# Sudaraka88/LDWeaver

Hardware: AMD Instinct MI355X
Metric: MI SNP-pairs/sec (higher is better)
Workload: dtype i8

## Files before the change

ldweaver_amd/csrc/ldw_apx.hip:

```cpp
#include <algorithm>
#include <cmath>
#include <cstdlib>
#include <cstring>

#include "ldw_apx.h"
#include "ldw_dev.h"

using namespace ldw;

namespace ldw {

namespace {
constexpr int64_t APX_PROD_CAP = 12000;
struct ProdTable {
    std::vector<int32_t> val;
    std::vector<uint8_t> a, b;
    ProdTable() {
        std::vector<std::pair<int32_t, std::pair<uint8_t, uint8_t>>> all;
        for (int x = 0; x <= 127; ++x)
            for (int y = x; y <= 127; ++y) all.push_back({x * y, {(uint8_t)x, (uint8_t)y}});
        std::sort(all.begin(), all.end());
        for (auto &e : all)
            if (val.empty() || val.back() != e.first) {
                val.push_back(e.first);
// ... 724 lines not shown
                for (int i = 0; i < MT; ++i)
#pragma unroll
                    for (int j = 0; j < NT; ++j)
#pragma unroll
                        for (int e = 0; e < 16; ++e) acc[i][j][e] = (int)((unsigned)acc[i][j][e] >> sh);
            }
        };
        exp_issue(wcur[1], 2 * m + 1);
        rescale(sh4.x);
        if (wave_live) kstep(tile0, 0);
        exp_finish(wdst + 32768);
        rescale(sh4.y);
        if (wave_live) kstep(tile0, 1);
        __syncthreads();
        if (m + 1 < P.M2) exp_issue(wnext[0], 2 * m + 2);
        rescale(sh4.z);
        if (wave_live) kstep(tile0 + 32768, 0);
        if (m + 1 < P.M2) exp_finish(wdst);
        rescale(sh4.w);
        if (wave_live) kstep(tile0 + 32768, 1);
        __syncthreads();
        wcur = wnext;
        wnext = wfar;
    }
    if (!wave_live) return;
    apx_gemm_epilogue<MT, NT>(P, acc, ty, tx, lane, s_tab, reinterpret_cast<uint8_t *>(s_tab + 64 * 64) + wave * 256);
}

#endif

int launch_apx_live_tiles(ldw_ctx *c, const ApxGemmArgs &P, hipStream_t st) {
    LDW_REQUIRE(P.fuse && P.skip_ctr && P.tile_list && P.n_live && P.RTpad % 128 == 0 && P.RFpad % 64 == 0 && P.tab && P.tab_nb == 64,
                LDW_ERR_ARG, "launch_apx_live_tiles: bad pruning arguments");
    hipLaunchKernelGGL(k_apx_live_tiles, dim3((unsigned)(P.RTpad / (32 * APX_MT))), dim3(256), 0, st, P);
    LDW_HIP(hipGetLastError());
    return LDW_OK;
}

int launch_gemm_apx(ldw_ctx *c, const ApxGemmArgs &P, hipStream_t st) {
    LDW_REQUIRE(P.RTpad % APX_TW == 0 && P.RFpad % APX_TW == 0 && P.M2 > 0, LDW_ERR_ARG, "launch_gemm_apx: padding violated (RT %d RF %d M2 %d)", P.RTpad,
                P.RFpad, P.M2);
    const size_t lds = APX_LUT_BYTES + (size_t)P.M2 * 256 + (P.fuse ? (size_t)P.tab_nb * P.tab_nb * 8 + 1024 : 0);
    LDW_REQUIRE(lds <= 65536, LDW_ERR_ARG, "launch_gemm_apx: %d positions do not fit the LDS digit arrays", P.M2 * 128);
    LDW_REQUIRE(!P.fuse || (P.tab_nb == 64 && P.bin_t && P.bin_f && P.tab && P.clean), LDW_ERR_ARG, "launch_gemm_apx: bad table arguments");
    static const int tile = [] {
        const char *e = exp_env("LDW_APX_TILE");
        return e ? atoi(e) : 42;
    }();
#ifdef LDW_EXPERIMENTS
    const int kern = apx_kernel_is_lds() ? 1 : 0;
    static const bool pipe = [] { const char *e = exp_env("LDW_APX_KERNEL"); return e && e[0] == 'p'; }();
    if (pipe && !P.fine && tile == 42) {
        const int ntx = P.RFpad / 64, nty = P.RTpad / 128;
        hipLaunchKernelGGL(gemm_apx_pipe_kernel, dim3((unsigned)((ntx + 1) / 2), (unsigned)((nty + 1) / 2)), dim3(256), lds, st, P);
        LDW_HIP(hipGetLastError());
        int64_t waves = 0;
        for (int ty = 0; ty < nty; ++ty) {
            if (!P.lower_only) waves += ntx;
            else for (int tx = 0; tx < ntx; ++tx) waves += (tx * 64 + 63 < ty * 128) ? 0 : 1;
        }
        c->gemm_stat[0] += 1;
        if (P.fuse) c->gemm_stat[5] += 1;
        c->gemm_stat[1] += 2.0 * (double)waves * 128 * 64 * ((double)P.M2 * 128.0);
        return LDW_OK;
    }
    const size_t lds2 = 2048 + (size_t)P.M2 * 256 + 2 * 32768 + (P.fuse ? (size_t)P.tab_nb * P.tab_nb * 8 + 8 * 256 : 0);
    if (kern == 1 && lds2 <= 160 * 1024 && tile == 42) {
        static bool attr_set = false;
        if (!attr_set) {
            LDW_HIP(hipFuncSetAttribute(reinterpret_cast<const void *>(gemm_apx_lds_kernel), hipFuncAttributeMaxDynamicSharedMemorySize, 160 * 1024));
            attr_set = true;
        }
        const int ntx = P.RFpad / 64, nty = P.RTpad / 128;
        hipLaunchKernelGGL(gemm_apx_lds_kernel, dim3((unsigned)((ntx + 3) / 4), (unsigned)((nty + 1) / 2)), dim3(512), lds2, st, P);
        LDW_HIP(hipGetLastError());
        int64_t waves = 0;
        for (int ty = 0; ty < nty; ++ty) {
            if (!P.lower_only) waves += ntx;
            else for (int tx = 0; tx < ntx; ++tx) waves += (tx * 64 + 63 < ty * 128) ? 0 : 1;
        }
        c->gemm_stat[0] += 1;
        if (P.fuse) c->gemm_stat[5] += 1;
        c->gemm_stat[1] += 2.0 * (double)waves * 128 * 64 * ((double)P.M2 * 128.0);
        return LDW_OK;
    }
#endif
#define LDW_APX_LAUNCH(MTv, NTv)                                                                                              \
    {                                                                                                                         \
        const int ntx = P.RFpad / (32 * NTv), nty = P.RTpad / (32 * MTv);                                                     \
        if (P.fine) hipLaunchKernelGGL((gemm_apx_kernel<MTv, NTv, true>), dim3((unsigned)((ntx + 1) / 2), (unsigned)((nty + 1) / 2)), dim3(256), lds, st, P); \
        else hipLaunchKernelGGL((gemm_apx_kernel<MTv, NTv, false>), dim3((unsigned)((ntx + 1) / 2), (unsigned)((nty + 1) / 2)), dim3(256), lds, st, P); \
    }
    if (P.skip_ctr) {
        LDW_REQUIRE(P.fuse && P.tile_list && P.n_live && P.RFpad % 64 == 0, LDW_ERR_ARG, "launch_gemm_apx: bad pruning arguments");
        const int tiles = (P.RTpad / (32 * APX_MT)) * (P.RFpad / 64), g = (tiles + 3) / 4;
        if (P.fine) hipLaunchKernelGGL((gemm_apx_kernel<APX_MT, 2, true, APX_WPS>), dim3((unsigned)g), dim3(256), lds, st, P);
        else hipLaunchKernelGGL((gemm_apx_kernel<APX_MT, 2, false, APX_WPS>), dim3((unsigned)g), dim3(256), lds, st, P);
    }
#ifdef LDW_EXPERIMENTS
    else if (tile == 22 && !P.fuse) LDW_APX_LAUNCH(2, 2)
    else if (tile == 33 && !P.fuse) {
        const int ntx = (P.RFpad + 95) / 96, nty = (P.RTpad + 95) / 96;
        if (P.fine) hipLaunchKernelGGL((gemm_apx_kernel<3, 3, true, 2>), dim3((unsigned)((ntx + 1) / 2), (unsigned)((nty + 1) / 2)), dim3(256), lds, st, P);
        else hipLaunchKernelGGL((gemm_apx_kernel<3, 3, false, 2>), dim3((unsigned)((ntx + 1) / 2), (unsigned)((nty + 1) / 2)), dim3(256), lds, st, P);
    }
    else if (tile == 224 && !P.fuse) {
        const int ntx = P.RFpad / 64, nty = P.RTpad / 64;
        if (P.fine) hipLaunchKernelGGL((gemm_apx_kernel<2, 2, true, 4>), dim3((unsigned)((ntx + 1) / 2), (unsigned)((nty + 1) / 2)), dim3(256), lds, st, P);
        else hipLaunchKernelGGL((gemm_apx_kernel<2, 2, false, 4>), dim3((unsigned)((ntx + 1) / 2), (unsigned)((nty + 1) / 2)), dim3(256), lds, st, P);
    }
    else if (tile == 24 && !P.fuse) LDW_APX_LAUNCH(2, 4)
    else if (tile == 32 && !P.fuse) {
        const int ntx = P.RFpad / 64, nty = (P.RTpad + 95) / 96;
        if (P.fine) hipLaunchKernelGGL((gemm_apx_kernel<3, 2, true, 3>), dim3((unsigned)((ntx + 1) / 2), (unsigned)((nty + 1) / 2)), dim3(256), lds, st, P);
        else hipLaunchKernelGGL((gemm_apx_kernel<3, 2, false, 3>), dim3((unsigned)((ntx + 1) / 2), (unsigned)((nty + 1) / 2)), dim3(256), lds, st, P);
    }
#endif
    else LDW_APX_LAUNCH(4, 2)
#undef LDW_APX_LAUNCH
    LDW_HIP(hipGetLastError());
    {
        const int tl = P.fuse ? 42 : tile;
        const int MTv = (P.fuse && P.skip_ctr) ? APX_MT : (tl == 22 || tl == 24 || tl == 224 ? 2 : (tl == 32 || tl == 33 ? 3 : 4)), NTv = tl == 24 ? 4 : (tl == 33 ? 3 : 2), TH = 32 * MTv, TWd = 32 * NTv;
        int64_t waves = 0;
        for (int ty = 0; ty * TH < P.RTpad; ++ty) {
            const int ntx = P.RFpad / TWd;
            if (!P.lower_only) waves += ntx;
            else for (int tx = 0; tx < ntx; ++tx) waves += (tx * TWd + TWd - 1 < ty * TH) ? 0 : 1;
        }
        c->gemm_stat[0] += 1;
        if (P.fuse) c->gemm_stat[5] += 1;
        c->gemm_stat[1] += 2.0 * (double)waves * TH * TWd * ((double)P.M2 * 128.0);
        if (P.fuse && P.skip_ctr) {
            c->apx_ops_per_wave = 2.0 * TH * TWd * ((double)P.M2 * 128.0);
            c->apx_waves_total += waves;
        }
    }
    return LDW_OK;
}

struct PairArgs {
    const uint64_t *Mbits;
    int64_t KW;
    int nwords, path, nseg;
    int seg_in_lds;
    const PopSeg *segs;
    const int32_t *wbeg, *row0;
    int32_t zero_row;
    int64_t *sums;
    EpiArgs A;
    unsigned long long *ghist;
};

template <int CA, int CB>
__device__ __forceinline__ void pair_sums_body(const PairArgs &P, int path, const int32_t *s_wbeg, const PopSeg *s_segs) {
    constexpr bool GENB = CA == 4 && CB == 4;
    const EpiArgs &A = P.A;
    const int sub = path * PAIR_SHARDS + (int)blockIdx.y;
    unsigned int n = A.pl_n[sub];
    n = n > A.pl_cap ? A.pl_cap : n;
    const int lane = threadIdx.x & 63;
    const PairEnt *list = A.pl_pairs + (int64_t)sub * A.pl_cap;
    constexpr int KW = 3, KS = 2;
    uint32_t smask[KW][KS];
    int64_t sV[KW][KS];
    bool more[KW];
#pragma unroll
    for (int k = 0; k < KW; ++k) {
        const int w = lane + 64 * k;
        int s0 = 0, s1 = 0;
        if (w < P.nwords) {
            s0 = s_wbeg[w] & 0x7FFFFFFF;
            s1 = s_wbeg[w + 1] & 0x7FFFFFFF;
        }
        more[k] = s1 - s0 > KS;
#pragma unroll
        for (int q = 0; q < KS; ++q) {
            const bool on = s0 + q < s1 && !more[k];
            smask[k][q] = on ? s_segs[s0 + q].mask : 0u;
            sV[k][q] = on ? s_segs[s0 + q].V : 0;
        }
    }
    for (unsigned int idx = blockIdx.x * 4u + (threadIdx.x >> 6); idx < n; idx += gridDim.x * 4u) {
        const PairEnt e = list[idx];
        const uint32_t era = (uint32_t)__builtin_amdgcn_readfirstlane((int)e.ra), erb = (uint32_t)__builtin_amdgcn_readfirstlane((int)e.rb);
        const int r0a = (int)(era & 0x1FFFFFFFu), na = (int)(era >> 29), r0b = (int)(erb & 0x1FFFFFFFu), nb = (int)(erb >> 29);
        const uint32_t *fr[CA], *tr[CB];
#pragma unroll
        for (int i = 0; i < CA; ++i) fr[i] = reinterpret_cast<const uint32_t *>(P.Mbits + (int64_t)(i < na ? r0a + i : P.zero_row) * P.KW);
#pragma unroll
        for (int j = 0; j < CB; ++j) tr[j] = reinterpret_cast<const uint32_t *>(P.Mbits + (int64_t)(j < nb ? r0b + j : P.zero_row) * P.KW);
        int64_t s[CB][CA];
#pragma unroll
        for (int j = 0; j < CB; ++j)
#pragma unroll
            for (int i = 0; i < CA; ++i) s[j][i] = 0;
        uint32_t f[KW][CA], tt[KW][CB];
#pragma unroll
        for (int k = 0; k < KW; ++k) {
            const int w = lane + 64 * k;
            const bool in = w < P.nwords;
#pragma unroll
            for (int i = 0; i < CA; ++i) f[k][i] = (in && (!GENB || i < na)) ? fr[i][w] : 0u;
#pragma unroll
            for (int j = 0; j < CB; ++j) tt[k][j] = (in && (!GENB || j < nb)) ? tr[j][w] : 0u;
        }
#pragma unroll
        for (int k = 0; k < KW; ++k) {
            if (more[k]) {
                const int w = lane + 64 * k;
                const int s0 = s_wbeg[w] & 0x7FFFFFFF, s1 = s_wbeg[w + 1] & 0x7FFFFFFF;
                for (int sg = s0; sg < s1; ++sg) {
                    const PopSeg seg = s_segs[sg];
#pragma unroll
                    for (int j = 0; j < CB; ++j)
#pragma unroll
                        for (int i = 0; i < CA; ++i)
                            if (!GENB || (i < na && j < nb)) s[j][i] += (int64_t)((uint64_t)__popc(f[k][i] & tt[k][j] & seg.mask) * (uint64_t)seg.V);
                }
            } else {
#pragma unroll
                for (int q2 = 0; q2 < KS; ++q2)
#pragma unroll
                    for (int j = 0; j < CB; ++j)
#pragma unroll
                        for (int i = 0; i < CA; ++i)
                            if (!GENB || (i < na && j < nb)) s[j][i] += (int64_t)((uint64_t)__popc(f[k][i] & tt[k][j] & smask[k][q2]) * (uint64_t)sV[k][q2]);
            }
        }
        for (int w = lane + 64 * KW; w < P.nwords; w += 64) {
            uint32_t f2[CA], t2[CB];
#pragma unroll
            for (int i = 0; i < CA; ++i) f2[i] = (!GENB || i < na) ? fr[i][w] : 0u;
#pragma unroll
            for (int j = 0; j < CB; ++j) t2[j] = (!GENB || j < nb) ? tr[j][w] : 0u;
            const int s0 = s_wbeg[w] & 0x7FFFFFFF, s1 = s_wbeg[w + 1] & 0x7FFFFFFF;
            for (int sg = s0; sg < s1; ++sg) {
                const PopSeg seg = s_segs[sg];
#pragma unroll
                for (int j = 0; j < CB; ++j)
#pragma unroll
                    for (int i = 0; i < CA; ++i)
                        if (!GENB || (i < na && j < nb)) s[j][i] += (int64_t)((uint64_t)__popc(f2[i] & t2[j] & seg.mask) * (uint64_t)seg.V);
            }
        }
#pragma unroll
        for (int j = 0; j < CB; ++j)
#pragma unroll
            for (int i = 0; i < CA; ++i) {
                int64_t v = s[j][i];
                if (!GENB || (i < na && j < nb)) {
#pragma unroll
                    for (int off = 32; off > 0; off >>= 1) v += __shfl_xor(v, off);
                }
                if (lane == 0) P.sums[((int64_t)sub * A.pl_cap + idx) * 16 + j * 4 + i] = v;
            }
    }
}

template <bool GEN>
__global__ __launch_bounds__(256) void k_pair_sums(PairArgs P) {
    extern __shared__ __attribute__((aligned(16))) uint8_t pop_smem[];
    int32_t *s_wbeg = reinterpret_cast<int32_t *>(pop_smem);
    PopSeg *s_segs = reinterpret_cast<PopSeg *>(pop_smem + (((size_t)P.nwords + 4) * 4 + 15) / 16 * 16);
    const int path = GEN ? 4 : (int)blockIdx.z;
    if (blockIdx.x * 4u >= P.A.pl_n[path * PAIR_SHARDS + (int)blockIdx.y]) return;
    if (P.seg_in_lds) {
        for (int i = threadIdx.x; i < P.nwords + 1; i += 256) s_wbeg[i] = P.wbeg[i];
        for (int i = threadIdx.x; i < P.nseg; i += 256) s_segs[i] = P.segs[i];
        __syncthreads();
    } else {
        s_wbeg = const_cast<int32_t *>(P.wbeg);
        s_segs = const_cast<PopSeg *>(P.segs);
    }
    if constexpr (GEN) {
        pair_sums_body<4, 4>(P, 4, s_wbeg, s_segs);
    } else {
        switch (path) {
            case 0: pair_sums_body<1, 1>(P, 0, s_wbeg, s_segs); break;
            case 1: pair_sums_body<2, 1>(P, 1, s_wbeg, s_segs); break;
            case 2: pair_sums_body<1, 2>(P, 2, s_wbeg, s_segs); break;
            default: pair_sums_body<2, 2>(P, 3, s_wbeg, s_segs); break;
        }
    }
}

template <int CA, int CB>
__device__ __forceinline__ void pair_sums_bits_body(const PairArgs &P, int path, const int64_t *sVT, int stride) {
    constexpr bool GENB = CA == 4 && CB == 4;
    const EpiArgs &A = P.A;
    const int sub = path * PAIR_SHARDS + (int)blockIdx.y;
    unsigned int n = A.pl_n[sub];
    n = n > A.pl_cap ? A.pl_cap : n;
    const int lane = threadIdx.x & 63;
    const PairEnt *list = A.pl_pairs + (int64_t)sub * A.pl_cap;
    for (unsigned int idx = blockIdx.x * 4u + (threadIdx.x >> 6); idx < n; idx += gridDim.x * 4u) {
        const PairEnt e = list[idx];
        const uint32_t era = (uint32_t)__builtin_amdgcn_readfirstlane((int)e.ra), erb = (uint32_t)__builtin_amdgcn_readfirstlane((int)e.rb);
        const int r0a = (int)(era & 0x1FFFFFFFu), na = (int)(era >> 29), r0b = (int)(erb & 0x1FFFFFFFu), nb = (int)(erb >> 29);
        const uint32_t *fr[CA], *tr[CB];
#pragma unroll
        for (int i = 0; i < CA; ++i) fr[i] = reinterpret_cast<const uint32_t *>(P.Mbits + (int64_t)(i < na ? r0a + i : P.zero_row) * P.KW);
#pragma unroll
        for (int j = 0; j < CB; ++j) tr[j] = reinterpret_cast<const uint32_t *>(P.Mbits + (int64_t)(j < nb ? r0b + j : P.zero_row) * P.KW);
        int64_t s[CB][CA];
#pragma unroll
        for (int j = 0; j < CB; ++j)
#pragma unroll
            for (int i = 0; i < CA; ++i) s[j][i] = 0;
        for (int w = lane; w < P.nwords; w += 64) {
            uint32_t f[CA], t[CB], uf = 0u, ut = 0u;
#pragma unroll
            for (int i = 0; i < CA; ++i) {
                f[i] = (!GENB || i < na) ? fr[i][w] : 0u;
                uf |= f[i];
            }
#pragma unroll
            for (int j = 0; j < CB; ++j) {
                t[j] = (!GENB || j < nb) ? tr[j][w] : 0u;
                ut |= t[j];
            }
            uint32_t u = uf & ut;
            while (u) {
                const int b = __builtin_ctz(u);
                u &= u - 1u;
                const int64_t v = sVT[b * stride + w];
#pragma unroll
                for (int j = 0; j < CB; ++j)
#pragma unroll
                    for (int i = 0; i < CA; ++i)
                        if (CA * CB == 1 || (((f[i] & t[j]) >> b) & 1u)) s[j][i] += v;
            }
        }
#pragma unroll
        for (int j = 0; j < CB; ++j)
#pragma unroll
            for (int i = 0; i < CA; ++i) {
                int64_t v = s[j][i];
                if (!GENB || (i < na && j < nb)) {
#pragma unroll
                    for (int off = 32; off > 0; off >>= 1) v += __shfl_xor(v, off);
                }
                if (lane == 0) P.sums[((int64_t)sub * A.pl_cap + idx) * 16 + j * 4 + i] = v;
            }
    }
}

template <bool GEN>
__global__ __launch_bounds__(256) void k_pair_sums_bits(PairArgs P, const int64_t *__restrict__ vpos, int stride) {
    extern __shared__ __attribute__((aligned(16))) uint8_t pop_smem[];
    int64_t *sVT = reinterpret_cast<int64_t *>(pop_smem);
    const int path = GEN ? 4 : (int)blockIdx.z;
    if (blockIdx.x * 4u >= P.A.pl_n[path * PAIR_SHARDS + (int)blockIdx.y]) return;
    for (int i = threadIdx.x; i < 32 * stride; i += 256) {
        const int b = i / stride, w = i - b * stride;
        sVT[i] = w < P.nwords ? vpos[32 * w + b] : 0;
    }
    __syncthreads();
    if constexpr (GEN) {
        pair_sums_bits_body<4, 4>(P, 4, sVT, stride);
    } else {
        switch (path) {
            case 0: pair_sums_bits_body<1, 1>(P, 0, sVT, stride); break;
            case 1: pair_sums_bits_body<2, 1>(P, 1, sVT, stride); break;
            case 2: pair_sums_bits_body<1, 2>(P, 2, sVT, stride); break;
            default: pair_sums_bits_body<2, 2>(P, 3, sVT, stride); break;
        }
    }
}

constexpr int PAIR_HWIN = 128;

template <int NA, int NB>
__device__ __forceinline__ void pair_mi_body(const PairArgs &P, int path, unsigned int *s_hist) {
    constexpr bool GEN = NA == 0;
    const EpiArgs &A = P.A;
    const EmitArgs &E = A.E;
    const int sub = path * PAIR_SHARDS + (int)blockIdx.y;
    unsigned int n = A.pl_n[sub];
    n = n > A.pl_cap ? A.pl_cap : n;
    const bool square = A.nf == A.nt;
    const PairEnt *list = A.pl_pairs + (int64_t)sub * A.pl_cap;
    const int lane = (int)(threadIdx.x & 63);
    for (unsigned int base = blockIdx.x * 256u + (threadIdx.x & ~63u); base < n; base += gridDim.x * 256u) {
        const unsigned int idx = base + (unsigned int)lane;
        bool valid = idx < n;
        uint32_t t = 0, q = 0;
        if (valid) {
            t = list[idx].t;
            q = list[idx].q;
        }
        const RowPack &RP = A.rowpack[t];
        valid = valid && RP.a_loc >= 0;
        bool cand = false;
        int bk = 0, seg = -1, a_loc = 0, b_loc = 0, sg = 0;
        double mi = 0.0;
        if (valid) {
            const RowSide R = RP.R;
            a_loc = RP.a_loc;
            const ColMeta M = A.colpack[q];
            b_loc = M.bl;
            sg = A.span ? M.ci.pad[0] : 0;
            const int64_t *sp = P.sums + ((int64_t)sub * A.pl_cap + idx) * 16;
            if constexpr (GEN) {
                mi = pair_mi<4, 4>(A, R, M, a_loc, b_loc, square, gacc_plain(sp, 1, 4));
            } else {
                mi = pair_mi_full<NA, NB>(A, R, M, a_loc, b_loc, square, gacc_plain(sp, 1, 4));
            }
            seg = pair_seg(a_loc, b_loc, E.lower_only);
            if (seg >= 0 && E.any_sr && col_is_sr(M.ci, a_loc)) {
                emit_pair_spec(E, M.ci, a_loc, b_loc, R.sa, M.sb, mi, P.ghist);
            } else if (seg >= 0 && E.do_lr && mi >= E.spec_lo) {
                bk = mi_bucket(mi);
                cand = bk >= E.spec_B;
            }
        }
        if (A.span) {
            for (int k = 0; k < A.span; ++k) {
                const bool mine = cand && sg == k;
                const unsigned long long mk = __ballot(mine);
                if (mk == 0ull) continue;
                const int leader = __builtin_ctzll(mk);
                unsigned long long pos = 0;
                if (lane == leader) pos = atomicAdd(A.sseg[k].n_cand, (unsigned long long)__popcll(mk));
                pos = __shfl(pos, leader);
                if (mine) {
                    pos += (unsigned long long)__popcll(mk & ((1ull << lane) - 1ull));
                    A.sseg[k].ckey[pos] = f64_key(mi);
                    A.sseg[k].cval[pos] = ((uint64_t)seg << 62) | ((uint64_t)a_loc + (uint64_t)b_loc * (uint64_t)E.nf);
                    const int w = bk - (E.spec_B > 0 ? E.spec_B : 0);
                    if (w < PAIR_HWIN) atomicAdd(&s_hist[k * PAIR_HWIN + w], 1u);
                    else atomicAdd(&A.sseg[k].ghist[bk], 1ull);
                }
            }
            continue;
        }
        const unsigned long long mk = __ballot(cand);
        if (mk == 0ull) continue;
        const int leader = __builtin_ctzll(mk);
        unsigned long long pos = 0;
        if (lane == leader) pos = atomicAdd(E.n_cand, (unsigned long long)__popcll(mk));
        pos = __shfl(pos, leader);
        if (cand) {
            pos += (unsigned long long)__popcll(mk & ((1ull << lane) - 1ull));
            E.ckey[pos] = f64_key(mi);
            E.cval[pos] = ((uint64_t)seg << 62) | ((uint64_t)a_loc + (uint64_t)b_loc * (uint64_t)E.nf);
            const int w = bk - (E.spec_B > 0 ? E.spec_B : 0);
            if (w < PAIR_HWIN) atomicAdd(&s_hist[w], 1u);
            else atomicAdd(&P.ghist[bk], 1ull);
        }
    }
}

__global__ __launch_bounds__(256) void k_pair_mi(PairArgs P) {
    __shared__ unsigned int s_hist[LDW_SPAN_MAX * PAIR_HWIN];
    for (int i = threadIdx.x; i < LDW_SPAN_MAX * PAIR_HWIN; i += 256) s_hist[i] = 0u;
    __syncthreads();
    switch (blockIdx.z) {
        case 0: pair_mi_body<1, 1>(P, 0, s_hist); break;
        case 1: pair_mi_body<2, 1>(P, 1, s_hist); break;
        case 2: pair_mi_body<1, 2>(P, 2, s_hist); break;
        case 3: pair_mi_body<2, 2>(P, 3, s_hist); break;
        default: pair_mi_body<0, 0>(P, 4, s_hist); break;
    }
    __syncthreads();
    const int hb0 = P.A.E.spec_B > 0 ? P.A.E.spec_B : 0;
    if (P.A.span) {
        for (int i = threadIdx.x; i < P.A.span * PAIR_HWIN; i += 256) {
            const int k = i / PAIR_HWIN, w = i - k * PAIR_HWIN;
            if (s_hist[i] != 0u && hb0 + w < NBINS) atomicAdd(&P.A.sseg[k].ghist[hb0 + w], (unsigned long long)s_hist[i]);
        }
        return;
    }
    if (threadIdx.x < PAIR_HWIN && s_hist[threadIdx.x] != 0u && hb0 + (int)threadIdx.x < NBINS)
        atomicAdd(&P.ghist[hb0 + threadIdx.x], (unsigned long long)s_hist[threadIdx.x]);
}

int launch_pairs_exact(ldw_ctx *c, const EpiArgs &A, unsigned long long *ghist, int64_t *sums, hipStream_t st) {
    PairArgs P;
    memset(&P, 0, sizeof(P));
    P.Mbits = c->Mbits.as<uint64_t>();
    P.KW = c->KW;
    P.nwords = (int)(c->KW * 2);
    P.nseg = c->n_pop_segs;
    P.segs = c->pop_segs.as<PopSeg>();
    P.wbeg = c->pop_wbeg.as<int32_t>();
    P.row0 = c->row0.as<int32_t>();
    P.zero_row = (int32_t)c->R;
    P.sums = sums;
    P.A = A;
    P.ghist = ghist;
    size_t lds = (((size_t)P.nwords + 4) * 4 + 15) / 16 * 16 + (size_t)P.nseg * sizeof(PopSeg);
    P.seg_in_lds = lds <= 60000 ? 1 : 0;
    if (!P.seg_in_lds) lds = 0;
    const int stride = (P.nwords + 31) / 32 * 32;
    const size_t lds_bits = (size_t)32 * stride * 8;
    const bool bits_off = getenv("LDW_NO_PAIR_BITS") != nullptr;
    const bool many_classes = !P.seg_in_lds || P.nseg >= 8 * P.nwords;
    if (many_classes && !bits_off && lds_bits <= 160 * 1024 && c->pop_vpos.p) {
        if (lds_bits > 64 * 1024 && !c->pair_bits_attr) {
            LDW_HIP(hipFuncSetAttribute(reinterpret_cast<const void *>(k_pair_sums_bits<false>), hipFuncAttributeMaxDynamicSharedMemorySize, 160 * 1024));
            LDW_HIP(hipFuncSetAttribute(reinterpret_cast<const void *>(k_pair_sums_bits<true>), hipFuncAttributeMaxDynamicSharedMemorySize, 160 * 1024));
            c->pair_bits_attr = true;
        }
        hipLaunchKernelGGL(k_pair_sums_bits<false>, dim3(256, PAIR_SHARDS, 4), dim3(256), lds_bits, st, P, c->pop_vpos.as<int64_t>(), stride);
        hipLaunchKernelGGL(k_pair_sums_bits<true>, dim3(256, PAIR_SHARDS, 1), dim3(256), lds_bits, st, P, c->pop_vpos.as<int64_t>(), stride);
    } else {
        static const unsigned gx_env = [] { const char *e = getenv("LDW_PAIR_GRID"); return e ? (unsigned)atoi(e) : 0u; }();
        hipLaunchKernelGGL(k_pair_sums<false>, dim3(gx_env ? gx_env : 512u, PAIR_SHARDS, 4), dim3(256), lds, st, P);
        hipLaunchKernelGGL(k_pair_sums<true>, dim3(gx_env ? gx_env : 1024u, PAIR_SHARDS, 1), dim3(256), lds, st, P);
    }
    hipLaunchKernelGGL(k_pair_mi, dim3(64, PAIR_SHARDS, PAIR_PATHS), dim3(256), 0, st, P);
    LDW_HIP(hipGetLastError());
    return LDW_OK;
}

}

namespace ldw {
void warm_apx() {
    hipFuncAttributes a;
    (void)hipFuncGetAttributes(&a, reinterpret_cast<const void *>(&k_pack_panel));
    (void)hipGetLastError();
}
}
```

ldweaver_amd/csrc/ldw_internal.h:

```cpp
#pragma once
#include <hip/hip_runtime.h>
#include <stdint.h>
#include <stdlib.h>
#include <string>
#include <atomic>
#include <memory>
#include <mutex>
#include <thread>
#include <vector>

#include "../../include/ldweaver_amd.h"

#define LDW_NSLOT 3

#ifdef LDW_EXPERIMENTS
#define LDW_HAS_EXPERIMENTS 1
#else
#define LDW_HAS_EXPERIMENTS 0
#endif

namespace ldw {

inline const char *exp_env(const char *name) {
#ifdef LDW_EXPERIMENTS
    return getenv(name);
#else
    (void)name;
    return nullptr;
#endif
}

void set_error(const char *fmt, ...);
int hip_fail(hipError_t e, const char *what, const char *file, int line);

#define LDW_HIP(call)                                                        \
    do {                                                                     \
        hipError_t e__ = (call);                                             \
        if (e__ != hipSuccess) return ldw::hip_fail(e__, #call, __FILE__, __LINE__); \
    } while (0)

#define LDW_REQUIRE(cond, code, ...)   \
    do {                               \
        if (!(cond)) {                 \
            ldw::set_error(__VA_ARGS__); \
            return (code);             \
        }                              \
    } while (0)

struct DevBuf {
    void *p = nullptr;
    size_t cap = 0;
    int reserve(size_t bytes);
    int reserve_keep(size_t bytes, size_t used, hipStream_t s);
    void release();
    template <class T> T *as() const { return reinterpret_cast<T *>(p); }
};

constexpr int TILE = 128;
constexpr int KSTEP = 128;
constexpr int NBINS = 4096;

struct BlockStat {
    int64_t n_lr_total = 0, n_lr_kept = 0, n_sr = 0;
    double disc_thresh = 0;
};
struct BlockTrace {
    int diag = 0, guess = -1, B_true = -1, margin = 0, path = 0 , missed = 0, probed = 0;
    long long n_cand = 0;
};

}

struct ldw_ctx {
    int device = 0;
    hipStream_t stream = nullptr;
    bool own_stream = true;
    hipEvent_t ev[6] = {nullptr, nullptr, nullptr, nullptr, nullptr, nullptr};
    double last_ms[4] = {0, 0, 0, 0};
    int engine = LDW_ENGINE_MFMA;

    int64_t L = 0, N = 0, Npad = 0;
    int64_t KW = 0;
    ldw::DevBuf states;
    ldw::DevBuf chars;
    int64_t cN = 0, cL = 0;
    void *fasta = nullptr;

    bool have_weights = false;
    int nlimbs = 5;
    int frac_bits = 0;
    double neff = 0;
    int64_t total_fixed = 0;
    ldw::DevBuf digits;
    ldw::DevBuf vfixed;
    std::vector<int64_t> h_vfixed;
    std::vector<int64_t> h_vfixed_hi;
    int64_t total_fixed_hi = 0;
    double lo_abs_sum = 0;
    int mixed = 1;

    std::vector<int32_t> h_seq_perm;
    ldw::DevBuf seq_perm;
    int path_mode = 0;
    int select_mode = 0;
    bool apx_ok = false;
    bool apx_fine = false;
    std::string apx_gate = "weights not set";
    ldw::DevBuf dig_a, dig_b;
    ldw::DevBuf apx_shift;
    int apx_e_last = 0;
    int apx_transitions = 0;
    double apx_lost_units = 0;
    double apx_delta = 0;
    std::vector<int64_t> h_vapx;
    ldw::DevBuf slot_papx;
    ldw::DevBuf pop_segs, pop_wbeg;
    ldw::DevBuf pop_vpos;
    bool pair_bits_attr = false;
    int n_pop_segs = 0, n_classes = 0;
    ldw::DevBuf panel[LDW_NSLOT][2];
    ldw::DevBuf Gapx[LDW_NSLOT];
    ldw::DevBuf tab11[2];
    double tab11_lo[2] = {0, 0};
    int tab11_cur[2] = {0, 0};
    int64_t tab11_builds = 0;
    float tab11_c = 0;
    int tab11_nb = 0;
    bool tab11_on = true;
    ldw::DevBuf pair_sums;
    ldw::DevBuf pairs[LDW_NSLOT];
    ldw::DevBuf sub_units[LDW_NSLOT], sub_packs[LDW_NSLOT], sub_bins[LDW_NSLOT], sub_live[LDW_NSLOT];
    ldw::DevBuf scr_live[LDW_NSLOT];
    ldw::DevBuf apx_bins[LDW_NSLOT], apx_clean[LDW_NSLOT];
    ldw::DevBuf apx_mini[LDW_NSLOT];
    ldw::DevBuf apx_units[LDW_NSLOT], apx_packs[LDW_NSLOT];
    int64_t apx_blocks = 0, apx_units_listed = 0, apx_pairs_listed = 0, probe_blocks = 0, generic_blocks = 0;
    bool prune = true;
    ldw::DevBuf apx_skip;
    double apx_ops_per_wave = 0;
    int64_t apx_waves_skipped = 0, apx_waves_total = 0;
    bool span_on = true;
    bool diag_split = false;
    bool span_corners = false;
    int span_max = 8;
    int64_t maybe_entries = 0;
    int64_t pair_list_overflows = 0, maybe_overflows = 0;
    bool maybe_off = false;
    int64_t span_items = 0, span_blocks = 0, span_fallbacks = 0;
    int64_t span_sr_subs = 0;
    bool early_sr = false;
    std::atomic<int64_t> sorted_blocks{0};
    std::mutex order_mtx;
    ldw::DevBuf snp_sup;
    double r_min = 0;
    struct OrderCache { std::vector<int32_t> idx, order; };
    std::vector<std::unique_ptr<OrderCache>> order_cache;

    bool have_meta = false;
    double g = 0;
    ldw::DevBuf r, uqe, POS, paint;
    std::vector<double> h_r;
    std::vector<int32_t> h_POS, h_paint;
    int32_t paint_min = 0, paint_max = 0;
    bool pos_sorted = true;
    bool pos_strict = true;
    ldw::DevBuf pos_slot;
    int64_t n_slots = 0;
    double sr_total_dist = -1;
    int64_t sr_total = -1;
    uint64_t sr_share_key = 0;
    int64_t sr_share_rows = -1;

    bool rows_ready = false;
    int64_t R = 0;
    ldw::DevBuf Mbits;
    ldw::DevBuf row0;
    ldw::DevBuf slot_meta;
    ldw::DevBuf slot_pfix;
    ldw::DevBuf slot_pfix_hi;
    bool hi_ready = false;
    ldw::DevBuf glo;
    ldw::DevBuf lo_rows;
    ldw::DevBuf packs;
    ldw::DevBuf counts;
    ldw::DevBuf pfix_state;
    std::vector<int32_t> h_row0;
    std::vector<uint32_t> h_slot_meta;
    std::vector<int32_t> h_counts;
    std::vector<int64_t> h_minor_w;
    std::vector<int32_t> h_span_bad;

    ldw::DevBuf G, G2, G3;
    ldw::DevBuf MIblk;
    ldw::DevBuf rowlist_f, rowlist_t, idx_f, idx_t, lrow_f, lrow_t, perm_f, perm_t;
    ldw::DevBuf epi_rest;
    ldw::DevBuf scr_units;
    ldw::DevBuf hist[LDW_NSLOT], cand_key[LDW_NSLOT], cand_val[LDW_NSLOT];
    ldw::DevBuf colcnt, cand_key2, cand_val2, scratch, small;
    ldw::DevBuf miss_key, miss_val;
    std::vector<uint8_t> ev_valid;
    ldw::DevBuf sel_bitmap, sel_chunks, sel_prefix;

    ldw::DevBuf sr_a, sr_b, sr_mi, lr_a, lr_b, lr_mi;
    int64_t n_sr = 0, n_lr = 0;
    int64_t blk_capacity = 0, blk_cursor = 0;

    void *lr_stream = nullptr;
    hipStream_t lr_st = nullptr;
    hipEvent_t lr_ev[64] = {};
    int64_t *lr_counts = nullptr;
    void *lr_pin = nullptr;
    size_t lr_pin_cap = 0;
    void *tsv_async = nullptr;
    void *pin_fetch = nullptr;
    size_t pin_fetch_cap = 0;
    ldw::DevBuf srm_pack, srm_key, srm_pack2, srm_key2, srm_pay, srm_pay2, srm_off, srm_q, srm_n, srm_md, srm_part, srm_shape, srm_cnt, srm_tmp;
    ldw::DevBuf srd_lower, srd_cur, srd_out, srd_seg;
    double ham_stat[8] = {0, 0, 0, 0, 0, 0, 0, 0};
    double gemm_stat[6] = {0, 0, 0, 0, 0, 0};
    ldw::DevBuf red_row, red_meta, red_srp, pool_a, pool_b, pool_mi, ar_key, ar_val, ar_key2, ar_val2, ar_off, ar_flags;
    int64_t n_red = 0, n_pool = 0;
    bool red_from_lr = false;
    int srm_S = 0, srm_nclust = 0;
    double srm_sr_dist = 0;

    hipStream_t copy_stream = nullptr, gemm_stream = nullptr;
    hipEvent_t ev_gemm[LDW_NSLOT] = {};
    bool overlap = true;
    void *pin[LDW_NSLOT + 1] = {};
    size_t pin_cap[LDW_NSLOT + 1] = {};
    ldw::DevBuf dstage[LDW_NSLOT + 1];
    hipEvent_t ev_up[LDW_NSLOT] = {}, ev_done[LDW_NSLOT] = {};
    bool done_recorded[LDW_NSLOT] = {};
    bool up_recorded[LDW_NSLOT] = {};
    void *pin_pick[LDW_NSLOT] = {};
    hipEvent_t ev_pick[LDW_NSLOT] = {};
    void *pin_lrc = nullptr;
    hipEvent_t ev_lrc = nullptr;
    bool lrc_recorded = false;
    bool fused = false;
    bool spec_seen[2] = {false, false};
    bool spec_probed[2] = {false, false};
    std::vector<hipEvent_t> ev_pool;
    int spec_hist[2][6] = {{0, 0, 0, 0, 0, 0}, {0, 0, 0, 0, 0, 0}};
    int spec_hist_n[2] = {0, 0};
    bool spec_small[2] = {false, false};
    int spec_B_next[2] = {-1, -1};
    int64_t spec_misses = 0, fused_blocks = 0, unfused_blocks = 0, screen_violations = 0, mixed_blocks = 0;
    int screen = 1;
    std::vector<ldw::BlockStat> stats;
    std::vector<int32_t> multi_owner;
    std::vector<ldw::BlockTrace> trace;
    std::thread *prep_thread = nullptr, *prep_thread2 = nullptr;
    int prep_rc = 0, prep_rc2 = 0;
    std::string prep_err, prep_err2;
};

namespace ldw {
int ensure_rows(ldw_ctx *ctx);
int set_dims(ldw_ctx *ctx, int64_t L, int64_t N);
int launch_hist(ldw_ctx *ctx, const int32_t *idx_f, int nf, const int32_t *idx_t, int nt, const int64_t *pfix_state,
                int quirk, int lower_only, double *MI);
int launch_gemm_bits(ldw_ctx *ctx, const uint64_t *Mbits, int64_t KW, const int32_t *rowlist_t, int RTpad, const int32_t *rowlist_f,
                     int RFpad, int64_t *G, int nlimbs, const int8_t *digits, int lower_only, hipStream_t stream = nullptr, int by0 = 0,
                     int by1 = -1,
                     const uint8_t *tile_mask = nullptr,
                     const uint32_t *tile_list = nullptr, int n_tile_list = 0);
int launch_cooc_popc(ldw_ctx *ctx, const int32_t *rowlist_t, int RTpad, const int32_t *rowlist_f, int RFpad, int64_t *G, int lower_only,
                     hipStream_t stream = nullptr);
int fill_rows_bits(ldw_ctx *ctx, const int32_t *d_rowinfo, int64_t R);
// ... 22 lines not shown
```

Before: 165.6 billion.

## Flatten pair-sum and MI work into persistent grids with grouped pairs per wave

Replaces the per-path/per-shard 3D grids for the pair-sum and MI kernels with a single flat work index. A wave-level prefix scan over all lists maps each index to a list and offset, and the grid is sized from the CU count. Each wave now handles several cheap pairs at once (4 for the 1x1 path, 2 for the mixed paths), prefetches the next group's entries, and reduces all sums with one transposing shuffle fold instead of separate full reductions. This targets idle blocks from uneven list sizes and shuffle overhead, but adds register pressure (launch bounds set to 4 waves) and per-iteration scan/ballot work.

```diff
diff --git a/ldweaver_amd/csrc/ldw_apx.hip b/ldweaver_amd/csrc/ldw_apx.hip
--- a/ldweaver_amd/csrc/ldw_apx.hip
+++ b/ldweaver_amd/csrc/ldw_apx.hip
@@ -900,119 +900,188 @@
     unsigned long long *ghist;
 };
 
-template <int CA, int CB>
-__device__ __forceinline__ void pair_sums_body(const PairArgs &P, int path, const int32_t *s_wbeg, const PopSeg *s_segs) {
+constexpr int PAIR_LISTS = PAIR_PATHS * PAIR_SHARDS;
+constexpr int PAIR_WG_PER_CU = 4;
+__host__ __device__ constexpr int pair_group(int path) { return path == 0 ? 4 : path == 4 ? 1 : 2; }
+
+template <int GCONST>
+__device__ __forceinline__ unsigned pair_group_scan(const EpiArgs &A, int l0, int nl, int lane, unsigned &n_l, unsigned &incl) {
+    n_l = 0u;
+    unsigned g = 0u;
+    if (lane < nl) {
+        n_l = A.pl_n[l0 + lane];
+        n_l = n_l > A.pl_cap ? A.pl_cap : n_l;
+        const unsigned G = (unsigned)(GCONST ? GCONST : pair_group((l0 + lane) / PAIR_SHARDS));
+        g = (n_l + G - 1u) / G;
+    }
+    incl = g;
+#pragma unroll
+    for (int off = 1; off < 64; off <<= 1) {
+        const unsigned o = __shfl_up(incl, off);
+        if (lane >= off) incl += o;
+    }
+    return (unsigned)__shfl((int)incl, 63);
+}
+__device__ __forceinline__ int pair_group_list(unsigned n_l, unsigned incl, unsigned gi, unsigned &g0, unsigned &n) {
+    const int l = __popcll(__ballot(incl <= gi));
+    g0 = l > 0 ? (unsigned)__shfl((int)incl, l - 1) : 0u;
+    n = (unsigned)__shfl((int)n_l, l);
+    return l;
+}
+
+template <int H>
+struct PairFold {
+    template <int NV>
+    __device__ __forceinline__ static void run(int64_t (&v)[NV], int lane, int off) {
+        const bool up = (lane & off) != 0;
+#pragma unroll
+        for (int k = 0; k < H; ++k) {
+            const int64_t send = up ? v[k] : v[k + H], keep = up ? v[k + H] : v[k];
+            v[k] = keep + __shfl_xor(send, off);
+        }
+        PairFold<H / 2>::run(v, lane, off >> 1);
+    }
+};
+template <>
+struct PairFold<0> {
+    template <int NV>
+    __device__ __forceinline__ static void run(int64_t (&v)[NV], int, int off) {
+        for (; off > 0; off >>= 1) v[0] += __shfl_xor(v[0], off);
+    }
+};
+
+constexpr int PS_KW = 3, PS_KS = 2;
+struct PairSegRegs {
+    uint32_t smask[PS_KW][PS_KS];
+    int64_t sV[PS_KW][PS_KS];
+    bool more[PS_KW];
+};
+
+template <int CA, int CB, int G>
+__device__ __forceinline__ void pair_sums_group(const PairArgs &P, int sub, unsigned i0, unsigned n, uint2 ent, const int32_t *s_wbeg,
+                                                const PopSeg *s_segs, const PairSegRegs &R, int lane) {
     constexpr bool GENB = CA == 4 && CB == 4;
-    const EpiArgs &A = P.A;
-    const int sub = path * PAIR_SHARDS + (int)blockIdx.y;
-    unsigned int n = A.pl_n[sub];
-    n = n > A.pl_cap ? A.pl_cap : n;
-    const int lane = threadIdx.x & 63;
-    const PairEnt *list = A.pl_pairs + (int64_t)sub * A.pl_cap;
-    constexpr int KW = 3, KS = 2;
-    uint32_t smask[KW][KS];
-    int64_t sV[KW][KS];
-    bool more[KW];
-#pragma unroll
-    for (int k = 0; k < KW; ++k) {
-        const int w = lane + 64 * k;
-        int s0 = 0, s1 = 0;
-        if (w < P.nwords) {
-            s0 = s_wbeg[w] & 0x7FFFFFFF;
-            s1 = s_wbeg[w + 1] & 0x7FFFFFFF;
-        }
-        more[k] = s1 - s0 > KS;
-#pragma unroll
-        for (int q = 0; q < KS; ++q) {
-            const bool on = s0 + q < s1 && !more[k];
-            smask[k][q] = on ? s_segs[s0 + q].mask : 0u;
-            sV[k][q] = on ? s_segs[s0 + q].V : 0;
-        }
-    }
-    for (unsigned int idx = blockIdx.x * 4u + (threadIdx.x >> 6); idx < n; idx += gridDim.x * 4u) {
-        const PairEnt e = list[idx];
-        const uint32_t era = (uint32_t)__builtin_amdgcn_readfirstlane((int)e.ra), erb = (uint32_t)__builtin_amdgcn_readfirstlane((int)e.rb);
-        const int r0a = (int)(era & 0x1FFFFFFFu), na = (int)(era >> 29), r0b = (int)(erb & 0x1FFFFFFFu), nb = (int)(erb >> 29);
-        const uint32_t *fr[CA], *tr[CB];
-#pragma unroll
-        for (int i = 0; i < CA; ++i) fr[i] = reinterpret_cast<const uint32_t *>(P.Mbits + (int64_t)(i < na ? r0a + i : P.zero_row) * P.KW);
-#pragma unroll
-        for (int j = 0; j < CB; ++j) tr[j] = reinterpret_cast<const uint32_t *>(P.Mbits + (int64_t)(j < nb ? r0b + j : P.zero_row) * P.KW);
-        int64_t s[CB][CA];
+    constexpr int KW = PS_KW, KS = PS_KS;
+    const uint32_t *fr[G][CA], *tr[G][CB];
+    int na[G], nb[G], la[G], lb[G];
+#pragma unroll
+    for (int g = 0; g < G; ++g) {
+        const uint32_t era = (uint32_t)__builtin_amdgcn_readlane((int)ent.x, g), erb = (uint32_t)__builtin_amdgcn_readlane((int)ent.y, g);
+        const int r0a = (int)(era & 0x1FFFFFFFu), r0b = (int)(erb & 0x1FFFFFFFu);
+        na[g] = (int)(era >> 29);
+        nb[g] = (int)(erb >> 29);
+        const bool valid = i0 + (unsigned)g < n;
+        la[g] = valid ? (GENB ? na[g] : CA) : 0;
+        lb[g] = valid ? (GENB ? nb[g] : CB) : 0;
+#pragma unroll
+        for (int i = 0; i < CA; ++i) fr[g][i] = reinterpret_cast<const uint32_t *>(P.Mbits + (int64_t)(i < na[g] ? r0a + i : P.zero_row) * P.KW);
+#pragma unroll
+        for (int j = 0; j < CB; ++j) tr[g][j] = reinterpret_cast<const uint32_t *>(P.Mbits + (int64_t)(j < nb[g] ? r0b + j : P.zero_row) * P.KW);
+    }
+    int64_t s[G][CB][CA];
+#pragma unroll
+    for (int g = 0; g < G; ++g)
 #pragma unroll
         for (int j = 0; j < CB; ++j)
 #pragma unroll
-            for (int i = 0; i < CA; ++i) s[j][i] = 0;
-        uint32_t f[KW][CA], tt[KW][CB];
+            for (int i = 0; i < CA; ++i) s[g][j][i] = 0;
+    uint32_t f[G][KW][CA], tt[G][KW][CB];
+#pragma unroll
+    for (int g = 0; g < G; ++g)
 #pragma unroll
         for (int k = 0; k < KW; ++k) {
             const int w = lane + 64 * k;
             const bool in = w < P.nwords;
 #pragma unroll
-            for (int i = 0; i < CA; ++i) f[k][i] = (in && (!GENB || i < na)) ? fr[i][w] : 0u;
-#pragma unroll
-            for (int j = 0; j < CB; ++j) tt[k][j] = (in && (!GENB || j < nb)) ? tr[j][w] : 0u;
-        }
-#pragma unroll
-        for (int k = 0; k < KW; ++k) {
-            if (more[k]) {
-                const int w = lane + 64 * k;
-                const int s0 = s_wbeg[w] & 0x7FFFFFFF, s1 = s_wbeg[w + 1] & 0x7FFFFFFF;
-                for (int sg = s0; sg < s1; ++sg) {
-                    const PopSeg seg = s_segs[sg];
-#pragma unroll
-                    for (int j = 0; j < CB; ++j)
-#pragma unroll
-                        for (int i = 0; i < CA; ++i)
-                            if (!GENB || (i < na && j < nb)) s[j][i] += (int64_t)((uint64_t)__popc(f[k][i] & tt[k][j] & seg.mask) * (uint64_t)seg.V);
-                }
-            } else {
-#pragma unroll
-                for (int q2 = 0; q2 < KS; ++q2)
-#pragma unroll
-                    for (int j = 0; j < CB; ++j)
-#pragma unroll
-                        for (int i = 0; i < CA; ++i)
-                            if (!GENB || (i < na && j < nb)) s[j][i] += (int64_t)((uint64_t)__popc(f[k][i] & tt[k][j] & smask[k][q2]) * (uint64_t)sV[k][q2]);
-            }
-        }
-        for (int w = lane + 64 * KW; w < P.nwords; w += 64) {
-            uint32_t f2[CA], t2[CB];
-#pragma unroll
-            for (int i = 0; i < CA; ++i) f2[i] = (!GENB || i < na) ? fr[i][w] : 0u;
-#pragma unroll
-            for (int j = 0; j < CB; ++j) t2[j] = (!GENB || j < nb) ? tr[j][w] : 0u;
+            for (int i = 0; i < CA; ++i) f[g][k][i] = (in && i < la[g]) ? fr[g][i][w] : 0u;
+#pragma unroll
+            for (int j = 0; j < CB; ++j) tt[g][k][j] = (in && j < lb[g]) ? tr[g][j][w] : 0u;
+        }
+#pragma unroll
+    for (int k = 0; k < KW; ++k) {
+        if (R.more[k]) {
+            const int w = lane + 64 * k;
             const int s0 = s_wbeg[w] & 0x7FFFFFFF, s1 = s_wbeg[w + 1] & 0x7FFFFFFF;
             for (int sg = s0; sg < s1; ++sg) {
                 const PopSeg seg = s_segs[sg];
 #pragma unroll
+                for (int g = 0; g < G; ++g)
+#pragma unroll
+                    for (int j = 0; j < CB; ++j)
+#pragma unroll
+                        for (int i = 0; i < CA; ++i)
+                            if (!GENB || (i < na[g] && j < nb[g])) s[g][j][i] += (int64_t)((uint64_t)__popc(f[g][k][i] & tt[g][k][j] & seg.mask) * (uint64_t)seg.V);
+            }
+        } else {
+#pragma unroll
+            for (int q2 = 0; q2 < KS; ++q2)
+#pragma unroll
+                for (int g = 0; g < G; ++g)
+#pragma unroll
+                    for (int j = 0; j < CB; ++j)
+#pragma unroll
+                        for (int i = 0; i < CA; ++i)
+                            if (!GENB || (i < na[g] && j < nb[g]))
+                                s[g][j][i] += (int64_t)((uint64_t)__popc(f[g][k][i] & tt[g][k][j] & R.smask[k][q2]) * (uint64_t)R.sV[k][q2]);
+        }
+    }
+    for (int w = lane + 64 * KW; w < P.nwords; w += 64) {
+        uint32_t f2[G][CA], t2[G][CB];
+#pragma unroll
+        for (int g = 0; g < G; ++g) {
+#pragma unroll
+            for (int i = 0; i < CA; ++i) f2[g][i] = i < la[g] ? fr[g][i][w] : 0u;
+#pragma unroll
+            for (int j = 0; j < CB; ++j) t2[g][j] = j < lb[g] ? tr[g][j][w] : 0u;
+        }
+        const int s0 = s_wbeg[w] & 0x7FFFFFFF, s1 = s_wbeg[w + 1] & 0x7FFFFFFF;
+        for (int sg = s0; sg < s1; ++sg) {
+            const PopSeg seg = s_segs[sg];
+#pragma unroll
+            for (int g = 0; g < G; ++g)
+#pragma unroll
                 for (int j = 0; j < CB; ++j)
 #pragma unroll
                     for (int i = 0; i < CA; ++i)
-                        if (!GENB || (i < na && j < nb)) s[j][i] += (int64_t)((uint64_t)__popc(f2[i] & t2[j] & seg.mask) * (uint64_t)seg.V);
-            }
-        }
+                        if (!GENB || (i < na[g] && j < nb[g])) s[g][j][i] += (int64_t)((uint64_t)__popc(f2[g][i] & t2[g][j] & seg.mask) * (uint64_t)seg.V);
+        }
+    }
+    constexpr int NV = G * CB * CA, RUN = 64 / NV;
+    static_assert(NV <= 64 && (NV & (NV - 1)) == 0, "the fold needs a power of two of at most 64 values");
+    int64_t v[NV];
+#pragma unroll
+    for (int g = 0; g < G; ++g)
 #pragma unroll
         for (int j = 0; j < CB; ++j)
 #pragma unroll
-            for (int i = 0; i < CA; ++i) {
-                int64_t v = s[j][i];
-                if (!GENB || (i < na && j < nb)) {
-#pragma unroll
-                    for (int off = 32; off > 0; off >>= 1) v += __shfl_xor(v, off);
-                }
-                if (lane == 0) P.sums[((int64_t)sub * A.pl_cap + idx) * 16 + j * 4 + i] = v;
-            }
-    }
+            for (int i = 0; i < CA; ++i) v[(g * CB + j) * CA + i] = s[g][j][i];
+    PairFold<NV / 2>::run(v, lane, 32);
+    if ((lane & (RUN - 1)) == 0) {
+        const int x = lane / RUN, g = x / (CB * CA), j = (x / CA) % CB, i = x % CA;
+        if (i0 + (unsigned)g < n) P.sums[((int64_t)sub * P.A.pl_cap + i0 + (unsigned)g) * 16 + j * 4 + i] = v[0];
+    }
+}
+
+__device__ __forceinline__ uint2 pair_group_ents(const EpiArgs &A, int l, unsigned i0, unsigned n, int lane) {
+    uint2 e = make_uint2(0u, 0u);
+    if (lane < pair_group(l / PAIR_SHARDS) && i0 + (unsigned)lane < n) {
+        const PairEnt *pe = A.pl_pairs + (int64_t)l * A.pl_cap + i0 + (unsigned)lane;
+        e = make_uint2(pe->ra, pe->rb);
+    }
+    return e;
 }
 
 template <bool GEN>
-__global__ __launch_bounds__(256) void k_pair_sums(PairArgs P) {
+__global__ __launch_bounds__(256, 4) void k_pair_sums(PairArgs P) {
+    constexpr int L0 = GEN ? 4 * PAIR_SHARDS : 0, NL = GEN ? PAIR_SHARDS : 4 * PAIR_SHARDS;
     extern __shared__ __attribute__((aligned(16))) uint8_t pop_smem[];
     int32_t *s_wbeg = reinterpret_cast<int32_t *>(pop_smem);
     PopSeg *s_segs = reinterpret_cast<PopSeg *>(pop_smem + (((size_t)P.nwords + 4) * 4 + 15) / 16 * 16);
-    const int path = GEN ? 4 : (int)blockIdx.z;
-    if (blockIdx.x * 4u >= P.A.pl_n[path * PAIR_SHARDS + (int)blockIdx.y]) return;
+    const EpiArgs &A = P.A;
+    const int lane = (int)(threadIdx.x & 63);
+    unsigned n_l, incl;
+    const unsigned total = pair_group_scan<0>(A, L0, NL, lane, n_l, incl);
+    if (blockIdx.x * 4u >= total) return;
     if (P.seg_in_lds) {
         for (int i = threadIdx.x; i < P.nwords + 1; i += 256) s_wbeg[i] = P.wbeg[i];
         for (int i = threadIdx.x; i < P.nseg; i += 256) s_segs[i] = P.segs[i];
@@ -1021,15 +1090,56 @@
         s_wbeg = const_cast<int32_t *>(P.wbeg);
         s_segs = const_cast<PopSeg *>(P.segs);
     }
-    if constexpr (GEN) {
-        pair_sums_body<4, 4>(P, 4, s_wbeg, s_segs);
-    } else {
-        switch (path) {
-            case 0: pair_sums_body<1, 1>(P, 0, s_wbeg, s_segs); break;
-            case 1: pair_sums_body<2, 1>(P, 1, s_wbeg, s_segs); break;
-            case 2: pair_sums_body<1, 2>(P, 2, s_wbeg, s_segs); break;
-            default: pair_sums_body<2, 2>(P, 3, s_wbeg, s_segs); break;
-        }
+    PairSegRegs R;
+#pragma unroll
+    for (int k = 0; k < PS_KW; ++k) {
+        const int w = lane + 64 * k;
+        int s0 = 0, s1 = 0;
+        if (w < P.nwords) {
+            s0 = s_wbeg[w] & 0x7FFFFFFF;
+            s1 = s_wbeg[w + 1] & 0x7FFFFFFF;
+        }
+        R.more[k] = s1 - s0 > PS_KS;
+#pragma unroll
+        for (int q = 0; q < PS_KS; ++q) {
+            const bool on = s0 + q < s1 && !R.more[k];
+            R.smask[k][q] = on ? s_segs[s0 + q].mask : 0u;
+            R.sV[k][q] = on ? s_segs[s0 + q].V : 0;
+        }
+    }
+    const unsigned nw = gridDim.x * 4u;
+    unsigned gi = blockIdx.x * 4u + (threadIdx.x >> 6);
+    if (gi >= total) return;
+    unsigned g0, n;
+    int l = L0 + pair_group_list(n_l, incl, gi, g0, n);
+    unsigned i0 = (gi - g0) * (unsigned)pair_group(l / PAIR_SHARDS);
+    uint2 ent = pair_group_ents(A, l, i0, n, lane);
+    for (;;) {
+        const unsigned gn = gi + nw;
+        unsigned g0n = 0u, nn = 0u, i0n = 0u;
+        int ln = 0;
+        uint2 entn = make_uint2(0u, 0u);
+        if (gn < total) {
+            ln = L0 + pair_group_list(n_l, incl, gn, g0n, nn);
+            i0n = (gn - g0n) * (unsigned)pair_group(ln / PAIR_SHARDS);
+            entn = pair_group_ents(A, ln, i0n, nn, lane);
+        }
+        if constexpr (GEN) {
+            pair_sums_group<4, 4, pair_group(4)>(P, l, i0, n, ent, s_wbeg, s_segs, R, lane);
+        } else {
+            switch (l / PAIR_SHARDS) {
+                case 0: pair_sums_group<1, 1, pair_group(0)>(P, l, i0, n, ent, s_wbeg, s_segs, R, lane); break;
+                case 1: pair_sums_group<2, 1, pair_group(1)>(P, l, i0, n, ent, s_wbeg, s_segs, R, lane); break;
+                case 2: pair_sums_group<1, 2, pair_group(2)>(P, l, i0, n, ent, s_wbeg, s_segs, R, lane); break;
+                default: pair_sums_group<2, 2, pair_group(3)>(P, l, i0, n, ent, s_wbeg, s_segs, R, lane); break;
+            }
+        }
+        if (gn >= total) break;
+        gi = gn;
+        l = ln;
+        i0 = i0n;
+        n = nn;
+        ent = entn;
     }
 }
 
@@ -1120,17 +1230,14 @@
 constexpr int PAIR_HWIN = 128;
 
 template <int NA, int NB>
-__device__ __forceinline__ void pair_mi_body(const PairArgs &P, int path, unsigned int *s_hist) {
+__device__ __forceinline__ void pair_mi_group(const PairArgs &P, int sub, unsigned int base, unsigned int n, unsigned int *s_hist) {
     constexpr bool GEN = NA == 0;
     const EpiArgs &A = P.A;
     const EmitArgs &E = A.E;
-    const int sub = path * PAIR_SHARDS + (int)blockIdx.y;
-    unsigned int n = A.pl_n[sub];
-    n = n > A.pl_cap ? A.pl_cap : n;
     const bool square = A.nf == A.nt;
     const PairEnt *list = A.pl_pairs + (int64_t)sub * A.pl_cap;
     const int lane = (int)(threadIdx.x & 63);
-    for (unsigned int base = blockIdx.x * 256u + (threadIdx.x & ~63u); base < n; base += gridDim.x * 256u) {
+    {
         const unsigned int idx = base + (unsigned int)lane;
         bool valid = idx < n;
         uint32_t t = 0, q = 0;
@@ -1181,10 +1288,10 @@
                     else atomicAdd(&A.sseg[k].ghist[bk], 1ull);
                 }
             }
-            continue;
+            return;
         }
         const unsigned long long mk = __ballot(cand);
-        if (mk == 0ull) continue;
+        if (mk == 0ull) return;
         const int leader = __builtin_ctzll(mk);
         unsigned long long pos = 0;
         if (lane == leader) pos = atomicAdd(E.n_cand, (unsigned long long)__popcll(mk));
@@ -1202,14 +1309,23 @@
 
 __global__ __launch_bounds__(256) void k_pair_mi(PairArgs P) {
     __shared__ unsigned int s_hist[LDW_SPAN_MAX * PAIR_HWIN];
+    const int lane = (int)(threadIdx.x & 63);
+    unsigned n_l, incl;
+    const unsigned total = pair_group_scan<64>(P.A, 0, PAIR_LISTS, lane, n_l, incl);
+    if (blockIdx.x * 4u >= total) return;
     for (int i = threadIdx.x; i < LDW_SPAN_MAX * PAIR_HWIN; i += 256) s_hist[i] = 0u;
     __syncthreads();
-    switch (blockIdx.z) {
-        case 0: pair_mi_body<1, 1>(P, 0, s_hist); break;
-        case 1: pair_mi_body<2, 1>(P, 1, s_hist); break;
-        case 2: pair_mi_body<1, 2>(P, 2, s_hist); break;
-        case 3: pair_mi_body<2, 2>(P, 3, s_hist); break;
-        default: pair_mi_body<0, 0>(P, 4, s_hist); break;
+    for (unsigned gi = blockIdx.x * 4u + (threadIdx.x >> 6); gi < total; gi += gridDim.x * 4u) {
+        unsigned g0, n;
+        const int l = pair_group_list(n_l, incl, gi, g0, n);
+        const unsigned base = (gi - g0) * 64u;
+        switch (l / PAIR_SHARDS) {
+            case 0: pair_mi_group<1, 1>(P, l, base, n, s_hist); break;
+            case 1: pair_mi_group<2, 1>(P, l, base, n, s_hist); break;
+            case 2: pair_mi_group<1, 2>(P, l, base, n, s_hist); break;
+            case 3: pair_mi_group<2, 2>(P, l, base, n, s_hist); break;
+            default: pair_mi_group<0, 0>(P, l, base, n, s_hist); break;
+        }
     }
     __syncthreads();
     const int hb0 = P.A.E.spec_B > 0 ? P.A.E.spec_B : 0;
@@ -1238,6 +1354,11 @@
     P.sums = sums;
     P.A = A;
     P.ghist = ghist;
+    if (c->n_cu <= 0) {
+        int cus = 256;
+        (void)hipDeviceGetAttribute(&cus, hipDeviceAttributeMultiprocessorCount, c->device);
+        c->n_cu = cus > 0 ? cus : 256;
+    }
     size_t lds = (((size_t)P.nwords + 4) * 4 + 15) / 16 * 16 + (size_t)P.nseg * sizeof(PopSeg);
     P.seg_in_lds = lds <= 60000 ? 1 : 0;
     if (!P.seg_in_lds) lds = 0;
@@ -1254,11 +1375,10 @@
         hipLaunchKernelGGL(k_pair_sums_bits<false>, dim3(256, PAIR_SHARDS, 4), dim3(256), lds_bits, st, P, c->pop_vpos.as<int64_t>(), stride);
         hipLaunchKernelGGL(k_pair_sums_bits<true>, dim3(256, PAIR_SHARDS, 1), dim3(256), lds_bits, st, P, c->pop_vpos.as<int64_t>(), stride);
     } else {
-        static const unsigned gx_env = [] { const char *e = getenv("LDW_PAIR_GRID"); return e ? (unsigned)atoi(e) : 0u; }();
-        hipLaunchKernelGGL(k_pair_sums<false>, dim3(gx_env ? gx_env : 512u, PAIR_SHARDS, 4), dim3(256), lds, st, P);
-        hipLaunchKernelGGL(k_pair_sums<true>, dim3(gx_env ? gx_env : 1024u, PAIR_SHARDS, 1), dim3(256), lds, st, P);
-    }
-    hipLaunchKernelGGL(k_pair_mi, dim3(64, PAIR_SHARDS, PAIR_PATHS), dim3(256), 0, st, P);
+        hipLaunchKernelGGL(k_pair_sums<false>, dim3((unsigned)(c->n_cu * PAIR_WG_PER_CU)), dim3(256), lds, st, P);
+        hipLaunchKernelGGL(k_pair_sums<true>, dim3((unsigned)(c->n_cu * PAIR_WG_PER_CU)), dim3(256), lds, st, P);
+    }
+    hipLaunchKernelGGL(k_pair_mi, dim3((unsigned)c->n_cu), dim3(256), 0, st, P);
     LDW_HIP(hipGetLastError());
     return LDW_OK;
 }
diff --git a/ldweaver_amd/csrc/ldw_internal.h b/ldweaver_amd/csrc/ldw_internal.h
--- a/ldweaver_amd/csrc/ldw_internal.h
+++ b/ldweaver_amd/csrc/ldw_internal.h
@@ -116,6 +116,7 @@
     ldw::DevBuf slot_papx;
     ldw::DevBuf pop_segs, pop_wbeg;
     ldw::DevBuf pop_vpos;
+    int n_cu = 0;
     bool pair_bits_attr = false;
     int n_pop_segs = 0, n_classes = 0;
     ldw::DevBuf panel[LDW_NSLOT][2];
```

Result: faster. 168.5 billion, median of 6 (+1.7%).
